# mobinasri/flagger

Hardware: AMD Instinct MI355X
Metric: coverage windows/sec through EM+decode; achieved HBM GB/s vs roofline (higher is better)
Workload: dtype f64

## Files before the change

### flagger_amd/_native.py

```python
from __future__ import annotations

import ctypes as C
import os

HF_NSTATES = 4
HF_MAXCOMP = 16
HF_MAXREGIONS = 64
HF_NKERNELS = 16
HF_MODEL_TRUNC_EXP_GAUSSIAN, HF_MODEL_GAUSSIAN, HF_MODEL_NEGATIVE_BINOMIAL = 0, 1, 2
HF_MODE_FULL, HF_MODE_FORWARD_ONLY = 0, 1
HF_ALGO_SCAN, HF_ALGO_SEQ = 0, 1
HF_STATS_CHUNKS, HF_STATS_ROWS = 0, 1
HF_EXCHANGE_CHUNKS, HF_EXCHANGE_RANKS = 0, 1
HF_TRANSPORT_RCCL, HF_TRANSPORT_LOOPBACK = 0, 1
HF_PROF_PASS = 0x80000000
HF_COUNT_WINDOWS, HF_COUNT_BASES = 0, 1
HF_OK, HF_E_ARG, HF_E_HIP, HF_E_SCALE, HF_E_NAN, HF_E_REGION, HF_E_NOGPU, HF_E_RETRY = 0, -1, -2, -3, -4, -5, -6, -7

LIB_PATH = os.path.join(os.path.dirname(os.path.abspath(__file__)), "csrc", "libhmmflagger_hip.so")
if os.environ.get("HF_LIBRARY_VARIANT"):
    LIB_PATH = os.path.join(os.path.dirname(LIB_PATH), "variants", "libhmmflagger_hip.%s.so" % os.environ["HF_LIBRARY_VARIANT"])


class hf_windows(C.Structure):
# ... 131 lines not shown
    sig("hf_comm_init_all", C.c_int, C.c_int, C.POINTER(C.c_int), C.POINTER(vp))
    sig("hf_comm_init_loopback", C.c_int, C.c_int, C.c_int, C.POINTER(vp))
    sig("hf_comm_destroy", None, vp)
    sig("hf_comm_rank", C.c_int, vp)
    sig("hf_comm_size", C.c_int, vp)
    sig("hf_comm_allgather", C.c_int, vp, vp, vp, i64, vp)
    sig("hf_comm_last_error", C.c_char_p)
    sig("hf_shard_bounds", C.c_int, C.POINTER(i64), i32, C.c_int, C.POINTER(i32))
    sig("hf_multi_create", C.c_int, C.POINTER(hf_windows), C.c_int, C.c_int, C.c_int, C.POINTER(C.c_int), C.c_int, C.c_int, C.c_int,
        C.POINTER(vp))
    sig("hf_multi_create_rank", C.c_int, C.POINTER(hf_windows), C.c_int, C.c_int, C.c_int, C.c_int, C.c_int, C.c_int, C.c_int, vp,
        C.POINTER(vp))
    sig("hf_multi_local_ctx", vp, vp)
    sig("hf_multi_local_first_window", i64, vp)
    sig("hf_multi_local_windows", i64, vp)
    sig("hf_multi_destroy", None, vp)
    sig("hf_multi_estep", C.c_int, vp, C.POINTER(hf_params), C.c_int, pd)
    sig("hf_multi_get_labels", C.c_int, vp, C.POINTER(C.c_int8))
    sig("hf_multi_get_posterior", C.c_int, vp, i64, i64, pd)
    sig("hf_multi_viterbi", C.c_int, vp, C.POINTER(hf_params), pd)
    sig("hf_multi_get_viterbi_labels", C.c_int, vp, C.POINTER(C.c_int8))
    sig("hf_multi_get_viterbi_chunk_log_probs", C.c_int, vp, pd)
    sig("hf_multi_world", C.c_int, vp)
    sig("hf_multi_comm_ranks", C.c_int, vp)
    sig("hf_multi_em_iterate", C.c_int, vp, vp, C.c_int, C.c_int, C.c_double, pd, C.POINTER(C.c_int))
    sig("hf_bind_rank_total", C.c_int, vp, vp, vp)
    sig("hf_multi_stats_len", i64, vp)
    sig("hf_multi_shard_windows", i64, vp, C.c_int)
    sig("hf_multi_shard_chunks", i32, vp, C.c_int)
    sig("hf_multi_rank_stats", C.c_int, vp, C.c_int, pd)
    sig("hf_multi_last_error", C.c_char_p)
    sig("hf_selftest_division", C.c_int, C.c_int, i64, pd, pd, pd, pd, C.POINTER(C.c_int32))
    sig("hf_selftest_exp", C.c_int, C.c_int, C.c_int64, C.POINTER(C.c_double), C.POINTER(C.c_double), C.POINTER(C.c_double), C.POINTER(C.c_double))
    sig("hfm_create", vp, C.c_int, C.c_int, C.POINTER(i32), C.c_int, C.c_int, C.c_int, C.c_int, pd, dbl, dbl)
    sig("hfm_copy", vp, vp)
    sig("hfm_destroy", None, vp)
    sig("hfm_n_regions", C.c_int, vp)
    sig("hfm_max_comps", C.c_int, vp)
    sig("hfm_model_type", C.c_int, vp)
    sig("hfm_max_high_mapq_ratio", dbl, vp)
    sig("hfm_min_high_mapq_ratio", dbl, vp)
    sig("hfm_min_highly_clipped_ratio", dbl, vp)
    sig("hfm_params", None, vp, C.POINTER(hf_params))
    sig("hfm_estimate", C.c_int, vp, pd, dbl)
    sig("hfm_loglikelihood", dbl, vp)
    sig("hfm_write_transition_tsv", C.c_int, vp, C.c_char_p)
    sig("hfm_write_emission_tsv", C.c_int, vp, C.c_char_p)
    sig("hfm_param_len", i64, vp)
    sig("hfm_get_param_vector", None, vp, pd)
    sig("hfm_set_param_vector", None, vp, pd)
    sig("hfm_best_collapsed_comps", C.c_int, C.POINTER(C.c_uint16), i64, C.POINTER(i32), C.c_int)
    sig("hfm_read_alpha_tsv", C.c_int, C.c_char_p, pd)
    sig("hfm_get_alpha", None, vp, pd)
    sig("hfm_set_alpha", C.c_int, vp, pd)
    sig("hfm_estimate_alpha", C.c_int, vp, pd, pd, C.POINTER(C.c_uint8), dbl, dbl, dbl)
    sig("hf_em_iterate", C.c_int, vp, vp, C.c_int, C.c_int, dbl, pd, C.POINTER(C.c_int), vp)
    sig("hfs_write_all_tables", C.c_int, C.POINTER(hfs_input), C.c_char_p, C.c_char_p, C.POINTER(C.c_char_p), C.c_int, dbl, C.c_int)
    sig("hfs_last_error", C.c_char_p)
    sig("hfm_scale_initial_means", None, vp, dbl)
    sig("hfm_set_max_coverage", None, vp, C.c_int)
    sig("hfm_squarem_create", vp, vp, vp, vp)
    sig("hfm_squarem_destroy", None, vp)
    sig("hfm_squarem_alpha", dbl, vp)
    sig("hfm_squarem_model_prime", vp, vp)
    sig("hfm_squarem_shrink", vp, vp)
    sig("hfm_is_feasible", C.c_int, vp)
# ... 44 lines not shown
```

### flagger_amd/csrc/hf_estep.hip

```cpp
#include "hf_device.h"
#include <hip/hip_ext.h>
#include "../../include/hmm_flagger_model.h"
#ifndef HF_SCAN_L
#define HF_SCAN_L 4
#endif
#include <string>
#include <algorithm>
#include <vector>
#include <cstring>
#include <cstdio>
#include <cmath>
#include <atomic>
#include <functional>
#include <condition_variable>
#include <mutex>
#include <memory>
#include <chrono>
#include <cstdlib>

#include <thread>
#include <unistd.h>
#include <immintrin.h>
static thread_local std::string g_err;

// ... 1804 lines not shown
    if (hf_device_count() <= 0) return set_err(HF_E_NOGPU, "hf_selftest_division: no HIP device");
    HIPCHK(hipSetDevice(device));
    double *da = nullptr, *dd = nullptr, *df = nullptr, *de = nullptr; int32_t* ds = nullptr;
    const size_t b = (size_t) (n ? n : 1) * 8;
    HIPCHK(hipMalloc((void**) &da, b)); HIPCHK(hipMalloc((void**) &dd, b)); HIPCHK(hipMalloc((void**) &df, b));
    HIPCHK(hipMalloc((void**) &de, b)); HIPCHK(hipMalloc((void**) &ds, b));
    HIPCHK(hipMemcpy(da, a, (size_t) n * 8, hipMemcpyHostToDevice)); HIPCHK(hipMemcpy(dd, d, (size_t) n * 8, hipMemcpyHostToDevice));
    if (n) hipLaunchKernelGGL(k_selftest_div, dim3((unsigned) ((n + 255) / 256)), dim3(256), 0, 0, n, da, dd, df, de, ds);
    HIPCHK(hipMemcpy(fast, df, (size_t) n * 8, hipMemcpyDeviceToHost)); HIPCHK(hipMemcpy(exact, de, (size_t) n * 8, hipMemcpyDeviceToHost));
    HIPCHK(hipMemcpy(safe, ds, (size_t) n * 4, hipMemcpyDeviceToHost));
    hipFree(da); hipFree(dd); hipFree(df); hipFree(de); hipFree(ds);
    return HF_OK;
}

__global__ void k_selftest_exp(int64_t n, const double* __restrict__ x, double* __restrict__ y) {
    const int64_t i = (int64_t) blockIdx.x * blockDim.x + threadIdx.x;
    if (i < n) y[i] = hf_exp(x[i]);
}
int hf_selftest_exp(int device, int64_t n, const double* x, double* dev_out, double* host_out, double* libm_out) {
    if (n < 0 || !x || !dev_out || !host_out || !libm_out) return set_err(HF_E_ARG, "hf_selftest_exp: bad argument");
    if (hf_device_count() <= 0) return set_err(HF_E_NOGPU, "hf_selftest_exp: no HIP device");
    HIPCHK(hipSetDevice(device));
    double *dx = nullptr, *dy = nullptr;
    const size_t b = (size_t) (n ? n : 1) * 8;
    HIPCHK(hipMalloc((void**) &dx, b)); HIPCHK(hipMalloc((void**) &dy, b));
    HIPCHK(hipMemcpy(dx, x, (size_t) n * 8, hipMemcpyHostToDevice));
    if (n) hipLaunchKernelGGL(k_selftest_exp, dim3((unsigned) ((n + 255) / 256)), dim3(256), 0, 0, n, dx, dy);
    HIPCHK(hipMemcpy(dev_out, dy, (size_t) n * 8, hipMemcpyDeviceToHost));
    hipFree(dx); hipFree(dy);
    for (int64_t i = 0; i < n; i++) { host_out[i] = hf_exp(x[i]); libm_out[i] = std::exp(x[i]); }
    return HF_OK;
}

int hf_last_kernel_ms(hf_ctx* ctx, float* ms) {
    if (!ctx || !ms || !ctx->pass.ev_valid) return set_err(HF_E_ARG, "hf_last_kernel_ms: nothing timed yet");
    Pass& ps = ctx->pass;
    HIPCHK(hipEventSynchronize(ps.ev1));
    HIPCHK(hipEventElapsedTime(ms, ps.ev0, ps.ev1));
    return HF_OK;
}

}

#include "hf_batch.h"


#include "hf_viterbi.h"
#include "hf_sample.h"

static bool dec_scan(const Track& tr) { return tr.algo == HF_ALGO_SCAN; }
static size_t dec_nrow(const Track& tr) { return dec_scan(tr) ? (size_t) tr.n_slots : (size_t) tr.N; }
static size_t dec_nseg(const Track& tr) { return dec_scan(tr) ? (size_t) tr.nseg : 0; }

template <class D, class F> static void dec_arrays(const Track& tr, D& d, bool score, F&& f) {
    const size_t G = dec_nseg(tr);
    f(d.d_params, tr.params_bytes); f(d.d_nbE, (size_t) tr.R * 4 * HF_NB_NX * 8); f(d.d_rows, dec_nrow(tr) * 128); f(d.d_flags, 4);
    if (dec_scan(tr)) {
        f(d.d_P, G * 16 * 64 * 8); f(d.d_S, G * 16 * 8); f(d.d_vin, G * 4 * 8);
        if (score) { f(d.d_PE, G * 64 * 4); f(d.d_SE, G * 4); f(d.d_vinE, G * 8); }
    }
}
template <class F> static void vit_arrays(const Track& tr, Viterbi& v, F&& f) {
    const size_t G = dec_nseg(tr);
    dec_arrays(tr, v, true, f);
    f(v.d_bp, dec_nrow(tr)); f(v.d_label, (size_t) tr.N); f(v.d_ll, (size_t) tr.C * 8); f(v.d_final, (size_t) tr.C);
    if (dec_scan(tr)) { f(v.d_lmap, G * 64); f(v.d_smap, G); f(v.d_sexit, G); }
// ... 886 lines not shown
```

### flagger_amd/csrc/hf_seg.h

```cpp
#pragma once
#include "hf_scan.h"

#define HF_SEG_LMAX 8
#define HF_SEG_SPLIT (64 * HF_SEG_LMAX)
#define HF_SEG_PSTAGE 24
#ifndef HF_SEG_OCC
#define HF_SEG_OCC 3
#endif


#if defined(__HIP_DEVICE_COMPILE__) && !defined(__GFX9__)
#error "hf_seg.h / hf_rows.h: the in-launch hand-offs rely on GFX9 (CDNA) vmcnt semantics; build with --offload-arch=gfx950"
#endif
#define HF_SEG_SPIN_MAX (1 << 16)
__device__ __forceinline__ void seg_xcu_store(double* p, double v) { __hip_atomic_store(p, v, __ATOMIC_RELAXED, __HIP_MEMORY_SCOPE_SYSTEM); }
__device__ __forceinline__ double seg_xcu_load(const double* p) { return __hip_atomic_load(p, __ATOMIC_RELAXED, __HIP_MEMORY_SCOPE_SYSTEM); }
#ifndef HF_SEG_WIDE
#define HF_SEG_WIDE 1
#endif
#ifndef HF_SEG_STAGGER
#define HF_SEG_STAGGER 0
#endif
#ifndef HF_SEG_STAGGER_PARTS
#define HF_SEG_STAGGER_PARTS 2
#endif
typedef unsigned hf_u32x4 __attribute__((ext_vector_type(4)));
__device__ __forceinline__ void seg_xcu_store_m4(double* p, const double m[16]) {
#if HF_SEG_WIDE
#pragma unroll
    for (int k = 0; k < 8; k++) {
        hf_u32x4 v;
        v.x = (unsigned) __double2loint(m[2 * k]); v.y = (unsigned) __double2hiint(m[2 * k]);
        v.z = (unsigned) __double2loint(m[2 * k + 1]); v.w = (unsigned) __double2hiint(m[2 * k + 1]);
        asm volatile("global_store_dwordx4 %0, %1, off sc0 sc1" :: "v"(p + 2 * k), "v"(v) : "memory");
    }
#else
#pragma unroll
    for (int k = 0; k < 16; k++) seg_xcu_store(p + k, m[k]);
#endif
}
__device__ __forceinline__ void seg_xcu_load_m4(const double* p, double m[16]) {
#if HF_SEG_WIDE
    hf_u32x4 v0, v1, v2, v3, v4, v5, v6, v7;
    asm volatile("global_load_dwordx4 %0, %8, off sc0 sc1\n\t"
                 "global_load_dwordx4 %1, %8, off offset:16 sc0 sc1\n\t"
                 "global_load_dwordx4 %2, %8, off offset:32 sc0 sc1\n\t"
                 "global_load_dwordx4 %3, %8, off offset:48 sc0 sc1\n\t"
                 "global_load_dwordx4 %4, %8, off offset:64 sc0 sc1\n\t"
                 "global_load_dwordx4 %5, %8, off offset:80 sc0 sc1\n\t"
                 "global_load_dwordx4 %6, %8, off offset:96 sc0 sc1\n\t"
                 "global_load_dwordx4 %7, %8, off offset:112 sc0 sc1\n\t"
                 "s_waitcnt vmcnt(0)"
                 : "=&v"(v0), "=&v"(v1), "=&v"(v2), "=&v"(v3), "=&v"(v4), "=&v"(v5), "=&v"(v6), "=&v"(v7) : "v"(p) : "memory");
    const hf_u32x4 v[8] = {v0, v1, v2, v3, v4, v5, v6, v7};
#pragma unroll
    for (int k = 0; k < 8; k++) { m[2 * k] = __hiloint2double((int) v[k].y, (int) v[k].x); m[2 * k + 1] = __hiloint2double((int) v[k].w, (int) v[k].z); }
#else
#pragma unroll
    for (int k = 0; k < 16; k++) m[k] = seg_xcu_load(p + k);
#endif
}

#define HF_SEG_TRACE_N 25
#ifdef HF_SEG_TRACE
__device__ unsigned long long* g_seg_trace = nullptr;
#define TR_DECL unsigned long long tr_acc[8] = {0, 0, 0, 0, 0, 0, 0, 0}; unsigned long long tr_t = clock64(); (void) tr_acc; (void) tr_t
#define TR_STAMP(k) do { if (BWD && g_seg_trace && lane == 0) g_seg_trace[(size_t) g * HF_SEG_TRACE_N + (k)] = clock64(); } while (0)
// ... 255 lines not shown

__device__ __forceinline__ void seg_suffix_side(M4& Q, int lane, double xs[16], double* s_T) {
    m4_scan_suffix_rows(Q, lane);
    if ((lane & 15) == 0 && lane > 0) {
        double2* dst = reinterpret_cast<double2*>(s_T) + ((lane >> 4) - 1) * 8;
#pragma unroll
        for (int k = 0; k < 8; k++) dst[k] = make_double2(Q.m[2 * k], Q.m[2 * k + 1]);
    }
    M4 X;
    m4_dpp0<HF_DPP_ROW_SHL(1)>(X, Q);
    m4_dpp_or_identity_fix(X, (lane & 15) != 15);
#pragma unroll
    for (int k = 0; k < 16; k++) xs[k] = X.m[k];
    __builtin_amdgcn_fence(__ATOMIC_RELEASE, "wavefront");
    __builtin_amdgcn_wave_barrier();
    __builtin_amdgcn_fence(__ATOMIC_ACQUIRE, "wavefront");
}
__device__ __forceinline__ void seg_suffix_apply(const double u[4], const double xs[16], int lane, const double* s_T, double bdir[4]) {
#pragma unroll
    for (int s = 0; s < 4; s++) bdir[s] = u[s];
    const int row = lane >> 4;
#pragma unroll
    for (int k = 3; k >= 1; k--) {
        double M[16], z[4] = {bdir[0], bdir[1], bdir[2], bdir[3]};
        const double2* src = reinterpret_cast<const double2*>(s_T) + (k - 1) * 8;
#pragma unroll
        for (int q = 0; q < 8; q++) { const double2 t2 = src[q]; M[2 * q] = t2.x; M[2 * q + 1] = t2.y; }
        v4_mul_left(z, M);
#pragma unroll
        for (int s = 0; s < 4; s++) bdir[s] = row < k ? z[s] : bdir[s];
    }
    v4_renorm(bdir);
    v4_mul_left(bdir, xs);
}

template <bool CACHED>
__device__ __forceinline__ void seg_lane_product(const RowFetch& F, const double* s_rows, int lane, int L, bool chunk_first, M4& Q) {
    double E[16];
    M4 A, R;
#define HF_ROW_TO_M4(dst) _Pragma("unroll") for (int k_ = 0; k_ < 16; k_++) (dst).m[k_] = E[HF_PS(k_ >> 2, k_ & 3)]
    int issued = 1;
    if constexpr (CACHED) {
        issued = F.nc + 1 < L ? F.nc + 1 : L;
        if (issued > 7) issued = 7;
        for (int st = 0; st < issued; st++) rows_issue(F, st);
    } else rows_issue(F, 0);
    auto step_rows = [&](int i) {
        if constexpr (CACHED) {
            rows_wait(issued - i - 1);
            rows_read(F, s_rows, i, lane, E);
            if (issued < L && (issued <= F.nc || issued - 1 <= i)) { rows_issue(F, issued); issued++; }
        } else {
            rows_wait(0);
            rows_read(F, s_rows, i, lane, E);
            if (i + 1 < L) rows_issue(F, i + 1);
        }
    };
    step_rows(0);
    HF_ROW_TO_M4(Q);
    if (chunk_first) m4_identity(Q);
    int i = 1;
#pragma unroll 1
    for (; i + 1 < L; i += 2) {
        step_rows(i);
        HF_ROW_TO_M4(A);
        m4_mul(R, Q, A);
// ... 4 lines not shown
    }
    if (i < L) {
        step_rows(i);
        HF_ROW_TO_M4(A);
        m4_mul(R, Q, A);
        Q = R;
        m4_renorm_tree(Q);
    }
#undef HF_ROW_TO_M4
}

__global__ void __launch_bounds__(64, 4) k_seg_prod(const SegDesc* __restrict__ sd, const int32_t* __restrict__ arow,
                                                    const double* __restrict__ lutA, double* __restrict__ Qs, double* __restrict__ Pseg) {
    extern __shared__ __attribute__((aligned(16))) double s_W[];
    double* __restrict__ blk = s_W;
    uint32_t* __restrict__ s_off = reinterpret_cast<uint32_t*>(s_W + 1024);
    const int g = blockIdx.x, lane = threadIdx.x;
    const SegDesc d = sd[g];
    const int L = d.L, a = lane * L;
    {
        int32_t rr[HF_SEG_LMAX];
        seg_load_arows(arow + d.t0, d.n, L, lane, d.ident_row, rr);
        seg_offsets_store(rr, L, lane, s_off);
    }
    const RowFetch F = rowfetch_init(lutA, s_off, blk, 0, lane);
    M4 Q;
    seg_lane_product<false>(F, blk, lane, L, a == 0 && d.k == 0, Q);
    {
        double2* __restrict__ dst = reinterpret_cast<double2*>(Qs) + (int64_t) g * 8 * 64 + lane;
#pragma unroll
        for (int k = 0; k < 8; k++) dst[k * 64] = make_double2(Q.m[2 * k], Q.m[2 * k + 1]);
    }
    if (d.nseg == 1) return;
    m4_scan_prefix(Q, lane);
    if (lane == 63) {
        double2* dst = reinterpret_cast<double2*>(Pseg + (int64_t) g * 16);
#pragma unroll
        for (int k = 0; k < 8; k++) dst[k] = make_double2(Q.m[2 * k], Q.m[2 * k + 1]);
    }
}

template <bool BWD, bool FUSED, bool CACHED>
__device__ __forceinline__ void seg_fb_body(const SegDesc* __restrict__ sd, const int32_t* __restrict__ arow,
                                            const double* __restrict__ lutA, const DevParams* __restrict__ P,
                                            const double* __restrict__ Qs, double* Pseg, unsigned* ready, unsigned epoch, unsigned wait_epoch,
                                            const int32_t* __restrict__ pos, double* __restrict__ recs, double* __restrict__ scale_s,
                                            int8_t* __restrict__ label, double* __restrict__ seg_ll,
                                            unsigned* __restrict__ flags, int32_t g0, int nc_arg,
                                            const int32_t* __restrict__ seg_of_block, int bx) {
    static_assert(FUSED || !CACHED, "cached row blocks: one-launch mode only");
    const int nc = CACHED ? nc_arg : 0;
    constexpr int LM = HF_SEG_LMAX;
    extern __shared__ __attribute__((aligned(16))) double s_W[];
    double* s_rows = s_W;
    double* blk = s_W + nc * 1024;
    uint32_t* __restrict__ s_off = reinterpret_cast<uint32_t*>(s_W + (nc + 1) * 1024);
    int8_t* __restrict__ s_lab = reinterpret_cast<int8_t*>(s_W + (nc + 1) * 1024) + 64 * LM * 4;
    double* s_P = blk;
    double* __restrict__ s_T = reinterpret_cast<double*>(s_lab);
    int g = bx + g0;
    const int lane = threadIdx.x;
    if (FUSED && BWD) KSTAMP(1);
    if (seg_of_block) { g = seg_of_block[g]; if (g < 0) return; }
    const SegDesc d = sd[g];
#if HF_SEG_STAGGER > 0
    if (FUSED && BWD) {
        const unsigned part = (unsigned) (((unsigned long long) blockIdx.x * HF_SEG_STAGGER_PARTS) / gridDim.x);
        if (part) {
            const unsigned long long t_end = clock64() + (unsigned long long) part * HF_SEG_STAGGER;
            while (clock64() < t_end) __builtin_amdgcn_s_sleep(16);
        }
    }
#endif
    const int L = d.L, n = d.n;
    const int a = lane * L;
    const int m = n - a < L ? (n - a > 0 ? n - a : 0) : L;
    const bool chunk_first = a == 0 && d.k == 0;
    unsigned bad = 0;
    double fin[4], bdir[4];
    TR_DECL;
    TR_STAMP(0);
#ifdef HF_SEG_TRACE
    if (BWD && g_seg_trace && lane == 0) g_seg_trace[(size_t) g * HF_SEG_TRACE_N + 24] = wall_clock64();
#endif
    const RowFetch F = rowfetch_init(lutA, s_off, s_rows, nc, lane);
    {
        int32_t rr[LM];
        seg_load_arows(arow + d.t0, n, L, lane, d.ident_row, rr);
        double v[4], u[4];
        {
            const double* __restrict__ A0 = lutA + (int64_t) d.chunk_slow0 * 16;
#pragma unroll
            for (int s = 0; s < 4; s++) v[s] = A0[HF_PS(0, s)];
        }
        const DevRegion* __restrict__ Rl = &P->reg[d.reg_last];
#pragma unroll
        for (int s = 0; s < 4; s++) u[s] = Rl->trans[s][4];
        M4 Q;
        double xv[16], xs[16];
        if constexpr (FUSED) {
            seg_offsets_store(rr, L, lane, s_off);
            seg_lane_product<CACHED>(F, s_rows, lane, L, chunk_first, Q);
            TR_STAMP(1);
            if (BWD) m4_park(Q, lane, blk);
            m4_scan_prefix(Q, lane);
            if (d.nseg > 1) {
                if (lane == 63) seg_xcu_store_m4(Pseg + (int64_t) g * 16, Q.m);
                asm volatile("s_waitcnt vmcnt(0)" ::: "memory");
                if (lane == 63) __hip_atomic_store(ready + g, epoch, __ATOMIC_RELAXED, __HIP_MEMORY_SCOPE_SYSTEM);
            }
            TR_STAMP(2);
            { M4 X_; m4_dpp0<HF_DPP_WAVE_SHR1>(X_, Q); m4_dpp_or_identity_fix(X_, lane > 0);
#pragma unroll
              for (int k = 0; k < 16; k++) xv[k] = X_.m[k]; }
            {
                const double sv = ((v[0] + v[1]) + v[2]) + v[3];
#pragma unroll
                for (int s = 0; s < 4; s++) v[s] /= sv;
            }
            if (BWD) v4_renorm(u);
            if (BWD) {
                m4_unpark(Q, lane, blk);
                seg_suffix_side(Q, lane, xs, s_T);
            }
            TR_STAMP(3);
            if (d.nseg > 1) {
                double Tm[16];
#pragma unroll
                for (int k = 0; k < 16; k++) Tm[k] = 0.0;
                int have_base = -1;
                auto stage = [&]() {
                    M4 T;
#pragma unroll
                    for (int k = 0; k < 16; k++) T.m[k] = Tm[k];
                    __builtin_amdgcn_s_waitcnt(0xC07F);
                    __builtin_amdgcn_wave_barrier();
                    m4_park(T, lane, blk);
                    __builtin_amdgcn_fence(__ATOMIC_RELEASE, "wavefront");
                    __builtin_amdgcn_wave_barrier();
                    __builtin_amdgcn_fence(__ATOMIC_ACQUIRE, "wavefront");
                };
                auto from_lane = [&](int src, double M[16]) {
                    const double2* __restrict__ row = reinterpret_cast<const double2*>(blk) + src * 8;
#pragma unroll
                    for (int k = 0; k < 8; k++) { const double2 t2 = row[(k + (src >> 1)) & 7]; M[2 * k] = t2.x; M[2 * k + 1] = t2.y; }
                };

                auto gather = [&](int base) {
                    if (base == have_base) return;
                    have_base = base;
                    const int q = base + lane;
                    if (q < d.nseg && q != d.k) {
                        const unsigned* r = ready + d.seg0 + q;
                        int spins = 0;
                        while (__hip_atomic_load(r, __ATOMIC_RELAXED, __HIP_MEMORY_SCOPE_SYSTEM) != wait_epoch) {
                            if (++spins > HF_SEG_SPIN_MAX) { bad |= HF_FLAG_SYNC; break; }
// ... 27 lines not shown
        }
        {
            const double2* __restrict__ src = reinterpret_cast<const double2*>(Qs) + (int64_t) g * 8 * 64 + lane;
#pragma unroll
            for (int k = 0; k < 8; k++) { const double2 q2 = src[k * 64]; Q.m[2 * k] = q2.x; Q.m[2 * k + 1] = q2.y; }
        }
        seg_offsets_store(rr, L, lane, s_off);
        TR_STAMP(1);
        if (d.nseg > 1) {
#pragma unroll
            for (int c = 0; c < (HF_SEG_PSTAGE * 8 + 63) / 64; c++) if (c * 64 + lane < nst * 8) reinterpret_cast<double2*>(s_P)[c * 64 + lane] = pst[c];
            __builtin_amdgcn_fence(__ATOMIC_RELEASE, "wavefront");
            __builtin_amdgcn_wave_barrier();
            __builtin_amdgcn_fence(__ATOMIC_ACQUIRE, "wavefront");
        }
        {
            const double sv = ((v[0] + v[1]) + v[2]) + v[3];
#pragma unroll
            for (int s = 0; s < 4; s++) v[s] /= sv;
        }
        for (int q = 0; q < d.k; q++) {
            if (q < HF_SEG_PSTAGE) v4_mul_right(v, s_P + q * 16); else v4_mul_right(v, Pseg + (int64_t) (d.seg0 + q) * 16);
            v4_renorm(v);
        }
        TR_STAMP(2);
        if (BWD) {
            v4_renorm(u);
            for (int q = d.nseg - 1; q > d.k; q--) {
                if (q < HF_SEG_PSTAGE) v4_mul_left(u, s_P + q * 16); else v4_mul_left(u, Pseg + (int64_t) (d.seg0 + q) * 16);
                v4_renorm(u);
            }
        }
        TR_STAMP(3);
        if (BWD) m4_park(Q, lane, blk);
        TR_STAMP(4);
        m4_scan_prefix(Q, lane);
        { M4 X_; m4_dpp0<HF_DPP_WAVE_SHR1>(X_, Q); m4_dpp_or_identity_fix(X_, lane > 0);
#pragma unroll
          for (int k = 0; k < 16; k++) xv[k] = X_.m[k]; }
        }
        if (true) v4_mul_right(v, xv);
        {
            const double su = ((v[0] + v[1]) + v[2]) + v[3];
#pragma unroll
            for (int s = 0; s < 4; s++) fin[s] = v[s] / su;
        }
        if (chunk_first) { fin[0] = 1.0; fin[1] = 0.0; fin[2] = 0.0; fin[3] = 0.0; }
        TR_STAMP(5);
        if (BWD) {
            if constexpr (!FUSED) {
                m4_unpark(Q, lane, blk);
                seg_suffix_side(Q, lane, xs, s_T);
            }
            seg_suffix_apply(u, xs, lane, s_T, bdir);
#pragma unroll
            for (int s = 0; s < 4; s++) asm volatile("" : "+v"(bdir[s]));
        }
    }
    TR_STAMP(6);
    double f[4] = {fin[0], fin[1], fin[2], fin[3]};
    double fs[LM][4], ss[LM];
    double A[16];
    double lm = 1.0, scl = 1.0;
    int le = 0;
    if (nc < L) rows_issue(F, nc);
    TR_RESET();
#pragma unroll
    for (int i = 0; i < LM; i++) {
        if (i < L) {
            if (i >= nc) rows_wait(0);
            rows_read(F, s_rows, i, lane, A);
            TR_LAP(0);
            if (i >= nc && i + 1 < L) rows_issue(F, i + 1);
            TR_LAP(1);
            if (i < m) {
                double nf[4];
#pragma unroll
                for (int s = 0; s < 4; s++) {
                    double acc = f[0] * A[HF_PS(0, s)];
#pragma unroll
                    for (int p = 1; p < 4; p++) acc = fma(f[p], A[HF_PS(p, s)], acc);
                    nf[s] = acc;
                }
                const double sc = ((nf[0] + nf[1]) + nf[2]) + nf[3];
                if (!(chunk_first && i == 0) && sc < 1e-50) bad |= HF_FLAG_SCALE;
// ... 129 lines not shown
#endif
    if (bad) atomicOr(flags, bad);
}

template <bool BWD, bool FUSED, bool CACHED = false>
__global__ void __launch_bounds__(64, HF_SEG_OCC) k_seg_fb(const SegDesc* __restrict__ sd, const int32_t* __restrict__ arow,
                                                           const double* __restrict__ lutA, const DevParams* __restrict__ P,
                                                           const double* __restrict__ Qs, double* Pseg, unsigned* ready, unsigned epoch, unsigned wait_epoch,
                                                           const int32_t* __restrict__ pos, double* __restrict__ recs, double* __restrict__ scale_s,
                                                           int8_t* __restrict__ label, double* __restrict__ seg_ll,
                                                           unsigned* __restrict__ flags, int32_t g0, int nc_arg,
                                                           const int32_t* __restrict__ seg_of_block) {
    seg_fb_body<BWD, FUSED, CACHED>(sd, arow, lutA, P, Qs, Pseg, ready, epoch, wait_epoch, pos, recs, scale_s, label, seg_ll, flags, g0, nc_arg,
                                    seg_of_block, (int) blockIdx.x);
}

struct SegFbModel {
    const double* lutA; const DevParams* P; const double* Qs; double* Pseg; unsigned* ready;
    double* recs; double* scale_s; int8_t* label; double* seg_ll; unsigned* flags;
};
#define HF_SEG_BATCH_MAX 64
struct SegFbBatch { int32_t model[HF_SEG_BATCH_MAX]; unsigned epoch[HF_SEG_BATCH_MAX]; unsigned wait_epoch[HF_SEG_BATCH_MAX]; };

template <bool BWD, bool FUSED, bool CACHED = false>
__global__ void __launch_bounds__(64, HF_SEG_OCC) k_seg_fb_batch(const SegDesc* __restrict__ sd, const int32_t* __restrict__ arow,
                                                                 const SegFbModel* __restrict__ tab, SegFbBatch bt,
                                                                 const int32_t* __restrict__ pos, int32_t g0, int nc_arg,
                                                                 const int32_t* __restrict__ seg_of_block) {
    const int y = (int) blockIdx.y;
    const SegFbModel& m = tab[bt.model[y]];
    seg_fb_body<BWD, FUSED, CACHED>(sd, arow, m.lutA, m.P, m.Qs, m.Pseg, m.ready, bt.epoch[y], bt.wait_epoch[y], pos, m.recs, m.scale_s, m.label,
                                    m.seg_ll, m.flags, g0, nc_arg, seg_of_block, (int) blockIdx.x);
}
```

### include/hmm_flagger_hip.h

```cpp
#ifndef HMM_FLAGGER_HIP_H
#define HMM_FLAGGER_HIP_H

#include <stdint.h>

#ifdef __cplusplus
extern "C" {
#endif

#define HF_NSTATES 4
#define HF_MAXCOMP 16
#define HF_MAXREGIONS 64

enum { HF_MODEL_TRUNC_EXP_GAUSSIAN = 0, HF_MODEL_GAUSSIAN = 1, HF_MODEL_NEGATIVE_BINOMIAL = 2 };
#define HF_NB_MAX_COVERAGE 250
enum { HF_MODE_FULL = 0,
       HF_MODE_FORWARD_ONLY = 1    };
enum { HF_ALGO_SCAN = 0,
       HF_ALGO_SEQ = 1             };

enum {
    HF_OK = 0,
    HF_E_ARG = -1,
    HF_E_HIP = -2,
    HF_E_SCALE = -3,
// ... 115 lines not shown

int hf_sample_capacity(const hf_ctx *ctx);
int hf_sample_paths(hf_ctx *ctx, const hf_params *p, int64_t first_sample, int n_samples, uint64_t seed, void *stream);
int hf_sample_finish(hf_ctx *ctx, void *stream);
int hf_get_sample_labels(hf_ctx *ctx, int k, int8_t *labels_host);

#define HF_BATCH_MAX_MODELS 1024
typedef struct hf_batch hf_batch;
int hf_batch_capacity(const hf_ctx *ctx);
int hf_batch_create(hf_ctx *ctx, int n_models, hf_batch **out);
void hf_batch_destroy(hf_batch *b);
int hf_batch_size(const hf_batch *b);
int hf_batch_shared_models(const hf_batch *b);
int64_t hf_batch_handoff(hf_batch *b, int model, uint32_t *epoch, uint32_t *ready_host, int64_t n);
int hf_batch_estep(hf_batch *b, const hf_params *p, const int32_t *models, int n_active, int mode, void *stream);
int hf_batch_finish(hf_batch *b, double *stats_host, int32_t *status, void *stream);
int hf_batch_get_labels(hf_batch *b, int model, int8_t *labels_host);
int hf_batch_get_posterior(hf_batch *b, int model, int64_t first, int64_t n, double *post_host);

int hf_last_kernel_ms(hf_ctx *ctx, float *ms);

#define HF_NKERNELS 16
enum { HF_K_TABLES = 0, HF_K_STATS_TILE = 4, HF_K_CHUNK_STATS, HF_K_REDUCE,
       HF_K_EMIT_ROWS, HF_K_FWD_SEQ, HF_K_BWD_SEQ, HF_K_PAIR_SUMS, HF_K_ROW_STATS, HF_K_ROWS_TOTAL, HF_K_SEG_PROD, HF_K_SEG_FB, HF_K_AROWS };
#define HF_PROF_PASS 0x80000000u
int hf_set_profiling(hf_ctx *ctx, unsigned kernel_mask);
int hf_set_profiling_stride(hf_ctx *ctx, int every_nth_pass);
int hf_kernel_times(hf_ctx *ctx, float ms[HF_NKERNELS]);
int hf_kernel_time_sums(hf_ctx *ctx, double sum_ms[HF_NKERNELS], int64_t launches[HF_NKERNELS]);
const char *hf_kernel_name(int k);

int hf_selftest_division(int device, int64_t n, const double *a, const double *d, double *fast, double *exact, int32_t *safe);
int hf_selftest_exp(int device, int64_t n, const double *x, double *dev_out, double *host_out, double *libm_out);

#ifdef __cplusplus
}
#endif
#endif
```

Before: 15.82 billion.

## Add MFMA-based 4x4 matrix prefix/suffix scan path behind HF_SEG_MFMA flag

Adds an alternative segment scan that parks per-lane 4x4 matrices in LDS and chains them with f64 4x4x4 MFMA instructions plus exponent renormalisation, replacing the DPP-based m4_scan_prefix and suffix side when HF_SEG_MFMA is set. The path is off by default, and selftest and timing entry points are added to compare the two variants. An s_nop is also inserted after each wide cross-XCU store, and that part runs on the default path, adding a small stall per store.

```diff
diff --git a/flagger_amd/_native.py b/flagger_amd/_native.py
--- a/flagger_amd/_native.py
+++ b/flagger_amd/_native.py
@@ -187,6 +187,8 @@
     sig("hf_multi_last_error", C.c_char_p)
     sig("hf_selftest_division", C.c_int, C.c_int, i64, pd, pd, pd, pd, C.POINTER(C.c_int32))
     sig("hf_selftest_exp", C.c_int, C.c_int, C.c_int64, C.POINTER(C.c_double), C.POINTER(C.c_double), C.POINTER(C.c_double), C.POINTER(C.c_double))
+    sig("hf_selftest_mfma_scan", C.c_int, C.c_int, i64, pd, pd, pd, pd, pd, pd)
+    sig("hf_selftest_scan_time", C.c_int, C.c_int, C.c_int, i64, C.c_int, C.c_int, C.c_int, C.c_int, pd, pd, pd, pd, pd, pd, C.POINTER(C.c_float))
     sig("hfm_create", vp, C.c_int, C.c_int, C.POINTER(i32), C.c_int, C.c_int, C.c_int, C.c_int, pd, dbl, dbl)
     sig("hfm_copy", vp, vp)
     sig("hfm_destroy", None, vp)
diff --git a/flagger_amd/csrc/hf_estep.hip b/flagger_amd/csrc/hf_estep.hip
--- a/flagger_amd/csrc/hf_estep.hip
+++ b/flagger_amd/csrc/hf_estep.hip
@@ -1860,6 +1860,52 @@
     return HF_OK;
 }
 
+static int selftest_scan_run(const char* who, int device, int variant, int64_t n_sets, int grid, int reps, int filler, int launches,
+                             const double* matrices_in, const double* v_in, const double* u_in, double* prefix_out, double* suffix_out,
+                             double* total_out, float* ms_per_launch) {
+    if (n_sets <= 0 || n_sets > (1 << 20) || grid <= 0 || reps <= 0 || launches <= 0 || filler < 0 || !matrices_in || !v_in || !u_in || !prefix_out ||
+        !suffix_out || !total_out)
+        return set_err(HF_E_ARG, std::string(who) + ": bad argument");
+    if (hf_device_count() <= 0) return set_err(HF_E_NOGPU, std::string(who) + ": no HIP device");
+    HIPCHK(hipSetDevice(device));
+    double *dm = nullptr, *dv = nullptr, *du = nullptr, *dp = nullptr, *dsf = nullptr, *dt = nullptr, *dsink = nullptr;
+    const size_t n = (size_t) n_sets;
+    HIPCHK(hipMalloc((void**) &dm, n * 64 * 16 * 8)); HIPCHK(hipMalloc((void**) &dv, n * 4 * 8)); HIPCHK(hipMalloc((void**) &du, n * 4 * 8));
+    HIPCHK(hipMalloc((void**) &dp, n * 64 * 4 * 8)); HIPCHK(hipMalloc((void**) &dsf, n * 64 * 4 * 8)); HIPCHK(hipMalloc((void**) &dt, n * 16 * 8));
+    HIPCHK(hipMalloc((void**) &dsink, 64 * 8));
+    HIPCHK(hipMemcpy(dm, matrices_in, n * 64 * 16 * 8, hipMemcpyHostToDevice));
+    HIPCHK(hipMemcpy(dv, v_in, n * 4 * 8, hipMemcpyHostToDevice)); HIPCHK(hipMemcpy(du, u_in, n * 4 * 8, hipMemcpyHostToDevice));
+    hipEvent_t e0, e1;
+    HIPCHK(hipEventCreate(&e0)); HIPCHK(hipEventCreate(&e1));
+    const size_t lds = 8192 + 512;
+    for (int l = 0; l <= launches; l++) {
+        if (l == 1) HIPCHK(hipEventRecord(e0, 0));
+        if (variant) hipLaunchKernelGGL(k_selftest_scan<true>, dim3((unsigned) grid), dim3(64), lds, 0, (int) n_sets, dm, dv, du, dp, dsf, dt, reps, filler, dsink);
+        else hipLaunchKernelGGL(k_selftest_scan<false>, dim3((unsigned) grid), dim3(64), lds, 0, (int) n_sets, dm, dv, du, dp, dsf, dt, reps, filler, dsink);
+    }
+    HIPCHK(hipEventRecord(e1, 0));
+    HIPCHK(hipEventSynchronize(e1));
+    float ms = 0.f;
+    HIPCHK(hipEventElapsedTime(&ms, e0, e1));
+    if (ms_per_launch) *ms_per_launch = ms / (float) launches;
+    HIPCHK(hipMemcpy(prefix_out, dp, n * 64 * 4 * 8, hipMemcpyDeviceToHost)); HIPCHK(hipMemcpy(suffix_out, dsf, n * 64 * 4 * 8, hipMemcpyDeviceToHost));
+    HIPCHK(hipMemcpy(total_out, dt, n * 16 * 8, hipMemcpyDeviceToHost));
+    hipEventDestroy(e0); hipEventDestroy(e1);
+    hipFree(dm); hipFree(dv); hipFree(du); hipFree(dp); hipFree(dsf); hipFree(dt); hipFree(dsink);
+    return HF_OK;
+}
+
+int hf_selftest_mfma_scan(int device, int64_t n_sets, const double* matrices_in, const double* v_in, const double* u_in, double* prefix_out,
+                          double* suffix_out, double* total_out) {
+    return selftest_scan_run("hf_selftest_mfma_scan", device, 1, n_sets, (int) n_sets, 1, 0, 1, matrices_in, v_in, u_in, prefix_out, suffix_out, total_out, nullptr);
+}
+
+int hf_selftest_scan_time(int device, int variant, int64_t n_sets, int grid, int reps, int filler, int launches, const double* matrices_in,
+                          const double* v_in, const double* u_in, double* prefix_out, double* suffix_out, double* total_out, float* ms_per_launch) {
+    return selftest_scan_run("hf_selftest_scan_time", device, variant, n_sets, grid, reps, filler, launches, matrices_in, v_in, u_in, prefix_out, suffix_out,
+                             total_out, ms_per_launch);
+}
+
 int hf_last_kernel_ms(hf_ctx* ctx, float* ms) {
     if (!ctx || !ms || !ctx->pass.ev_valid) return set_err(HF_E_ARG, "hf_last_kernel_ms: nothing timed yet");
     Pass& ps = ctx->pass;
diff --git a/flagger_amd/csrc/hf_seg.h b/flagger_amd/csrc/hf_seg.h
--- a/flagger_amd/csrc/hf_seg.h
+++ b/flagger_amd/csrc/hf_seg.h
@@ -32,7 +32,7 @@
         hf_u32x4 v;
         v.x = (unsigned) __double2loint(m[2 * k]); v.y = (unsigned) __double2hiint(m[2 * k]);
         v.z = (unsigned) __double2loint(m[2 * k + 1]); v.w = (unsigned) __double2hiint(m[2 * k + 1]);
-        asm volatile("global_store_dwordx4 %0, %1, off sc0 sc1" :: "v"(p + 2 * k), "v"(v) : "memory");
+        asm volatile("global_store_dwordx4 %0, %1, off sc0 sc1\n\ts_nop 1" :: "v"(p + 2 * k), "v"(v) : "memory");
     }
 #else
 #pragma unroll
@@ -354,6 +354,119 @@
     }
     v4_renorm(bdir);
     v4_mul_left(bdir, xs);
+}
+
+#ifndef HF_SEG_MFMA
+#define HF_SEG_MFMA 0
+#endif
+__device__ __forceinline__ void seg_lds_sync() {
+    __builtin_amdgcn_fence(__ATOMIC_RELEASE, "wavefront");
+    __builtin_amdgcn_wave_barrier();
+    __builtin_amdgcn_fence(__ATOMIC_ACQUIRE, "wavefront");
+}
+__device__ __forceinline__ double mq_mfma(double a, double b) { return __builtin_amdgcn_mfma_f64_4x4x4f64(a, b, 0.0, 0, 0, 0); }
+__device__ __forceinline__ double mq_renorm(double x) {
+    unsigned h = (unsigned) __double2hiint(x), t;
+    t = (unsigned) __builtin_amdgcn_update_dpp(0, (int) h, 0xB1, 0xf, 0xf, true); h = t > h ? t : h;
+    t = (unsigned) __builtin_amdgcn_update_dpp(0, (int) h, 0x4E, 0xf, 0xf, true); h = t > h ? t : h;
+    { const auto r = __builtin_amdgcn_permlane16_swap(h, h, false, false); h = r[0] > r[1] ? r[0] : r[1]; }
+    { const auto r = __builtin_amdgcn_permlane32_swap(h, h, false, false); h = r[0] > r[1] ? r[0] : r[1]; }
+    const int be = (int) ((h >> 20) & 0x7ffu);
+    int ne = be ? 1022 - be : 0;
+    asm volatile("" : "+v"(ne));
+    return ldexp(x, ne);
+}
+__device__ __forceinline__ void mq_park(const M4& Q, int lane, double* blk) {
+    const int q = lane & 15, b = lane >> 4;
+    const int z = ((b & 2) ? 5 : 0) ^ (q & 7);
+    double2* row = reinterpret_cast<double2*>(blk) + (4 * q + b) * 8;
+#pragma unroll
+    for (int k = 0; k < 8; k++) row[k ^ z] = make_double2(Q.m[2 * k], Q.m[2 * k + 1]);
+}
+struct MqLane { int b, en, et; };
+__device__ __forceinline__ MqLane mq_lane(int lane) {
+    const int j = lane & 3, i = lane >> 4;
+    MqLane c; c.b = (lane >> 2) & 3; c.en = i * 4 + j; c.et = j * 4 + i;
+    return c;
+}
+__device__ __forceinline__ double mq_read(const double* blk, int b, int q, int e) {
+    int idx = 64 * q + ((16 * b + (e ^ ((b & 2) ? 10 : 0))) ^ ((q & 7) << 1));
+    asm volatile("" : "+v"(idx));
+    return blk[idx];
+}
+__device__ __forceinline__ void mq_store_lane(double* blk, int l, int e, double x) { blk[16 * l + (e ^ (((l >> 1) & 7) << 1))] = x; }
+__device__ __forceinline__ void mq_unpark(double X[16], int lane, const double* blk) {
+    const double2* row = reinterpret_cast<const double2*>(blk) + lane * 8;
+    const int r = (lane >> 1) & 7;
+#pragma unroll
+    for (int k = 0; k < 8; k++) { const double2 d = row[k ^ r]; X[2 * k] = d.x; X[2 * k + 1] = d.y; }
+}
+template <bool SUF>
+__device__ __forceinline__ void mq_load(const double* blk, int lane, double qn[16], double tr[16]) {
+    const MqLane c = mq_lane(lane);
+#pragma unroll
+    for (int q = 0; q < 16; q++) {
+        if (q >= 1) qn[q] = mq_read(blk, c.b, q, c.en);
+        if (q == 0 || (SUF && q < 15)) tr[q] = mq_read(blk, c.b, q, c.et);
+    }
+}
+template <bool XV>
+__device__ __forceinline__ void seg_prefix_mfma(const double qn[16], double tr0, int lane, double* blk, double* s_aux, double Tm[16]) {
+    const MqLane c = mq_lane(lane);
+    double d = tr0;
+    if (XV) {
+        mq_store_lane(blk, 16 * c.b, c.et, c.en == c.et ? 1.0 : 0.0);
+        mq_store_lane(blk, 16 * c.b + 1, c.et, d);
+    }
+#pragma unroll
+    for (int q = 1; q < 16; q++) {
+        d = mq_mfma(qn[q], d);
+        if (!(q & 1) || q == 15) d = mq_renorm(d);
+        if (XV && q < 15) mq_store_lane(blk, 16 * c.b + q + 1, c.et, d);
+    }
+    s_aux[16 * ((c.b + 1) & 3) + c.et] = d;
+    seg_lds_sync();
+    double c2t = mq_mfma(s_aux[32 + c.en], s_aux[16 + c.et]);
+    const double u23 = mq_mfma(s_aux[48 + c.et], s_aux[c.en]);
+    const double r2 = s_aux[48 + c.en];
+    c2t = mq_renorm(c2t);
+    const double c3 = mq_renorm(mq_mfma(c2t, r2));
+    const double t = mq_renorm(mq_mfma(c2t, u23));
+    seg_lds_sync();
+    if (c.b == 0) { s_aux[c.en] = t; s_aux[32 + c.et] = c2t; s_aux[48 + c.en] = c3; }
+    seg_lds_sync();
+#pragma unroll
+    for (int k = 0; k < 16; k++) Tm[k] = s_aux[k];
+}
+__device__ __forceinline__ void seg_prefix_xv(int lane, const double* blk, const double* s_aux, double xv[16]) {
+    const int row = lane >> 4;
+    const double* Cb = row ? s_aux + 16 * row : blk;
+    M4 C, X, R;
+    __builtin_amdgcn_sched_barrier(0);
+#pragma unroll
+    for (int k = 0; k < 16; k++) C.m[k] = Cb[k];
+    mq_unpark(X.m, lane, blk);
+    m4_mul(R, C, X);
+#pragma unroll
+    for (int k = 0; k < 16; k++) { xv[k] = R.m[k]; asm volatile("" : "+v"(xv[k])); }
+    seg_lds_sync();
+    __builtin_amdgcn_sched_barrier(0);
+}
+__device__ __forceinline__ void seg_suffix_mfma(double qn15, const double tr[16], int lane, double* blk, double* s_T, double xs[16]) {
+    const MqLane c = mq_lane(lane);
+    double d = qn15;
+    mq_store_lane(blk, 16 * c.b + 15, c.en, c.en == c.et ? 1.0 : 0.0);
+    mq_store_lane(blk, 16 * c.b + 14, c.en, d);
+#pragma unroll
+    for (int q = 14; q >= 0; q--) {
+        d = mq_mfma(tr[q], d);
+        if (q & 1) d = mq_renorm(d);
+        if (q >= 1) mq_store_lane(blk, 16 * c.b + q - 1, c.en, d);
+    }
+    if (c.b >= 1) s_T[16 * (c.b - 1) + c.en] = d;
+    seg_lds_sync();
+    mq_unpark(xs, lane, blk);
+    seg_lds_sync();
 }
 
 template <bool CACHED>
@@ -424,7 +537,19 @@
         for (int k = 0; k < 8; k++) dst[k * 64] = make_double2(Q.m[2 * k], Q.m[2 * k + 1]);
     }
     if (d.nseg == 1) return;
+#if HF_SEG_MFMA
+    {
+        double* s_aux = reinterpret_cast<double*>(reinterpret_cast<int8_t*>(s_W + 1024) + 64 * HF_SEG_LMAX * 4);
+        double qn[16], tr[16];
+        mq_park(Q, lane, blk);
+        seg_lds_sync();
+        mq_load<false>(blk, lane, qn, tr);
+        seg_lds_sync();
+        seg_prefix_mfma<false>(qn, tr[0], lane, blk, s_aux, Q.m);
+    }
+#else
     m4_scan_prefix(Q, lane);
+#endif
     if (lane == 63) {
         double2* dst = reinterpret_cast<double2*>(Pseg + (int64_t) g * 16);
 #pragma unroll
@@ -490,21 +615,36 @@
         for (int s = 0; s < 4; s++) u[s] = Rl->trans[s][4];
         M4 Q;
         double xv[16], xs[16];
+#if HF_SEG_MFMA
+        double qn[16], tr[16];
+#endif
         if constexpr (FUSED) {
             seg_offsets_store(rr, L, lane, s_off);
             seg_lane_product<CACHED>(F, s_rows, lane, L, chunk_first, Q);
             TR_STAMP(1);
+#if HF_SEG_MFMA
+            mq_park(Q, lane, blk);
+            seg_lds_sync();
+            mq_load<BWD>(blk, lane, qn, tr);
+            seg_lds_sync();
+            seg_prefix_mfma<true>(qn, tr[0], lane, blk, s_T, Q.m);
+#else
             if (BWD) m4_park(Q, lane, blk);
             m4_scan_prefix(Q, lane);
+#endif
             if (d.nseg > 1) {
                 if (lane == 63) seg_xcu_store_m4(Pseg + (int64_t) g * 16, Q.m);
                 asm volatile("s_waitcnt vmcnt(0)" ::: "memory");
                 if (lane == 63) __hip_atomic_store(ready + g, epoch, __ATOMIC_RELAXED, __HIP_MEMORY_SCOPE_SYSTEM);
             }
             TR_STAMP(2);
+#if HF_SEG_MFMA
+            seg_prefix_xv(lane, blk, s_T, xv);
+#else
             { M4 X_; m4_dpp0<HF_DPP_WAVE_SHR1>(X_, Q); m4_dpp_or_identity_fix(X_, lane > 0);
 #pragma unroll
               for (int k = 0; k < 16; k++) xv[k] = X_.m[k]; }
+#endif
             {
                 const double sv = ((v[0] + v[1]) + v[2]) + v[3];
 #pragma unroll
@@ -512,8 +652,12 @@
             }
             if (BWD) v4_renorm(u);
             if (BWD) {
+#if HF_SEG_MFMA
+                seg_suffix_mfma(qn[15], tr, lane, blk, s_T, xs);
+#else
                 m4_unpark(Q, lane, blk);
                 seg_suffix_side(Q, lane, xs, s_T);
+#endif
             }
             TR_STAMP(3);
             if (d.nseg > 1) {
@@ -607,12 +751,22 @@
             }
         }
         TR_STAMP(3);
+#if HF_SEG_MFMA
+        mq_park(Q, lane, blk);
+        seg_lds_sync();
+        mq_load<BWD>(blk, lane, qn, tr);
+        seg_lds_sync();
+        TR_STAMP(4);
+        seg_prefix_mfma<true>(qn, tr[0], lane, blk, s_T, Q.m);
+        seg_prefix_xv(lane, blk, s_T, xv);
+#else
         if (BWD) m4_park(Q, lane, blk);
         TR_STAMP(4);
         m4_scan_prefix(Q, lane);
         { M4 X_; m4_dpp0<HF_DPP_WAVE_SHR1>(X_, Q); m4_dpp_or_identity_fix(X_, lane > 0);
 #pragma unroll
           for (int k = 0; k < 16; k++) xv[k] = X_.m[k]; }
+#endif
         }
         if (true) v4_mul_right(v, xv);
         {
@@ -624,8 +778,12 @@
         TR_STAMP(5);
         if (BWD) {
             if constexpr (!FUSED) {
+#if HF_SEG_MFMA
+                seg_suffix_mfma(qn[15], tr, lane, blk, s_T, xs);
+#else
                 m4_unpark(Q, lane, blk);
                 seg_suffix_side(Q, lane, xs, s_T);
+#endif
             }
             seg_suffix_apply(u, xs, lane, s_T, bdir);
 #pragma unroll
@@ -821,3 +979,72 @@
     seg_fb_body<BWD, FUSED, CACHED>(sd, arow, m.lutA, m.P, m.Qs, m.Pseg, m.ready, bt.epoch[y], bt.wait_epoch[y], pos, m.recs, m.scale_s, m.label,
                                     m.seg_ll, m.flags, g0, nc_arg, seg_of_block, (int) blockIdx.x);
 }
+
+template <bool MFMA>
+__global__ void __launch_bounds__(64, HF_SEG_OCC) k_selftest_scan(int n_sets, const double* __restrict__ mats, const double* __restrict__ v_in,
+                                                                   const double* __restrict__ u_in, double* __restrict__ pre, double* __restrict__ suf,
+                                                                   double* __restrict__ tot, int reps, int filler, double* __restrict__ sink) {
+    extern __shared__ __attribute__((aligned(16))) double s_W[];
+    double* blk = s_W;
+    double* s_aux = s_W + 1024;
+    const int lane = threadIdx.x, set = (int) (blockIdx.x % (unsigned) n_sets);
+    if (filler && (blockIdx.x & 3) == 3) {
+        double a0 = 1.0 + lane * 1e-9, a1 = 0.5, a2 = 0.25, a3 = 0.125;
+        for (int r = 0; r < reps * filler; r++) { a0 = fma(a0, 0.999, 1e-3); a1 = fma(a1, 0.999, 1e-3); a2 = fma(a2, 0.999, 1e-3); a3 = fma(a3, 0.999, 1e-3); }
+        if (a0 + a1 + a2 + a3 == 123.0) sink[lane] = a0;
+        return;
+    }
+    double v[4], u[4], fin[4], bdir[4];
+#pragma unroll
+    for (int s = 0; s < 4; s++) { v[s] = v_in[set * 4 + s]; u[s] = u_in[set * 4 + s]; fin[s] = 0.0; bdir[s] = 0.0; }
+#define HF_UNIT(x, n) do { double mx_ = (x)[0];                                                    \
+        _Pragma("unroll") for (int k_ = 1; k_ < (n); k_++) mx_ = (x)[k_] > mx_ ? (x)[k_] : mx_;       \
+        if (mx_ > 0.0) { _Pragma("unroll") for (int k_ = 0; k_ < (n); k_++) (x)[k_] /= mx_; } } while (0)
+    auto store_total = [&](double* Tm) {
+        HF_UNIT(Tm, 16);
+#pragma unroll
+        for (int k = 0; k < 16; k++) tot[(int64_t) set * 16 + k] = Tm[k];
+    };
+#pragma unroll 1
+    for (int r = 0; r < reps; r++) {
+        int ln = lane;
+        asm volatile("" : "+v"(ln));
+        M4 W;
+        {
+            const double2* src = reinterpret_cast<const double2*>(mats) + ((int64_t) set * 64 + ln) * 8;
+#pragma unroll
+            for (int k = 0; k < 8; k++) { const double2 d = src[k]; W.m[2 * k] = d.x; W.m[2 * k + 1] = d.y; }
+        }
+        double xv[16], xs[16], Tm[16];
+        if constexpr (MFMA) {
+            double qn[16], tr[16];
+            mq_park(W, ln, blk);
+            seg_lds_sync();
+            mq_load<true>(blk, ln, qn, tr);
+            seg_lds_sync();
+            seg_prefix_mfma<true>(qn, tr[0], ln, blk, s_aux, Tm);
+            if (r == reps - 1 && lane == 63) store_total(Tm);
+            seg_prefix_xv(ln, blk, s_aux, xv);
+            seg_suffix_mfma(qn[15], tr, ln, blk, s_aux, xs);
+        } else {
+            m4_park(W, ln, blk);
+            m4_scan_prefix(W, ln);
+#pragma unroll
+            for (int k = 0; k < 16; k++) Tm[k] = W.m[k];
+            if (r == reps - 1 && lane == 63) store_total(Tm);
+            { M4 X_; m4_dpp0<HF_DPP_WAVE_SHR1>(X_, W); m4_dpp_or_identity_fix(X_, ln > 0);
+#pragma unroll
+              for (int k = 0; k < 16; k++) xv[k] = X_.m[k]; }
+            m4_unpark(W, ln, blk);
+            seg_suffix_side(W, ln, xs, s_aux);
+        }
+#pragma unroll
+        for (int s = 0; s < 4; s++) fin[s] = v[s];
+        v4_mul_right(fin, xv);
+        seg_suffix_apply(u, xs, ln, s_aux, bdir);
+        seg_lds_sync();
+    }
+    HF_UNIT(fin, 4); HF_UNIT(bdir, 4);
+#pragma unroll
+    for (int s = 0; s < 4; s++) { pre[((int64_t) set * 64 + lane) * 4 + s] = fin[s]; suf[((int64_t) set * 64 + lane) * 4 + s] = bdir[s]; }
+}
diff --git a/include/hmm_flagger_hip.h b/include/hmm_flagger_hip.h
--- a/include/hmm_flagger_hip.h
+++ b/include/hmm_flagger_hip.h
@@ -171,6 +171,10 @@
 
 int hf_selftest_division(int device, int64_t n, const double *a, const double *d, double *fast, double *exact, int32_t *safe);
 int hf_selftest_exp(int device, int64_t n, const double *x, double *dev_out, double *host_out, double *libm_out);
+int hf_selftest_mfma_scan(int device, int64_t n_sets, const double *matrices_in, const double *v_in, const double *u_in, double *prefix_out,
+                          double *suffix_out, double *total_out);
+int hf_selftest_scan_time(int device, int variant, int64_t n_sets, int grid, int reps, int filler, int launches, const double *matrices_in,
+                          const double *v_in, const double *u_in, double *prefix_out, double *suffix_out, double *total_out, float *ms_per_launch);
 
 #ifdef __cplusplus
 }
```

Result: no change. 15.81 billion (median of 2 runs) (-0.0%).
